# sdrobert/pydrobert-pytorch

Hardware: AMD Instinct MI355X
Metric: utterances/sec (N=4096,T=512) error_rate+ctc_beam at 1/2/4/8 GPU (higher is better)
Workload: dtype f32

## Files before the change

pydrobert-pytorch_amd/csrc/ctc_frame.hpp:

```cpp
#pragma once
#include "wave_select.hpp"

namespace pdt {

#ifdef PDT_STAMPS
__device__ unsigned long long g_stamps[16];
__device__ unsigned long long *g_stamp_lds_dummy;
#define PDT_STAMP(ph)                                                        \
  do {                                                                       \
    const unsigned long long now_ = __builtin_readcyclecounter();           \
    pdt_stamp_acc[ph] += (unsigned)(now_ - stamp_last_);                     \
    stamp_last_ = now_;                                                      \
  } while (0)
#define PDT_STAMP_BEGIN unsigned long long stamp_last_ = __builtin_readcyclecounter()
#else
#define PDT_STAMP(ph) do {} while (0)
#define PDT_STAMP_BEGIN do {} while (0)
#endif

#ifdef PDT_STATS
__device__ unsigned long long g_stats[24];
#define PDT_STAT(i) do { if (lane_id() == 0) atomicAdd(&g_stats[i], 1ull); } while (0)
#else
#define PDT_STAT(i) do {} while (0)
#endif

#ifdef PDT_UTT_STATS
__device__ unsigned g_utt_stats[8192 * 4];
#define PDT_UTT(k, v) do { pdt_utt_acc[k] += (unsigned)(v); } while (0)
#else
#define PDT_UTT(k, v) do {} while (0)
#endif

constexpr int kMaxWidth = 32;

struct CtcArgs {
  const float *logits;
  int64_t lg_st, lg_sn, lg_sv;
  const int64_t *lens;
  int T, N, V, W, S;
  int64_t *y;
  int64_t *y_lens;
  float *y_probs;
  int2 *trie;
  int2 *ckpt;
  unsigned char *grow;
  int ckpt_shift, ckpt_count;
  int lds_per_wave, waves_per_wg;
  int exact_div;
  int no_lean_extra;
  int no_steady;
};

struct Beam {
  float nb, b;
  int last, len, node;
  unsigned isp;
  int origin = 0;
};

__device__ __forceinline__ u64 readlane_u64(u64 v, int l) {
  const unsigned lo = (unsigned)__builtin_amdgcn_readlane((int)(unsigned)v, l);
  const unsigned hi = (unsigned)__builtin_amdgcn_readlane((int)(unsigned)(v >> 32), l);
  return ((u64)hi << 32) | lo;
}
__device__ __forceinline__ float readlane_f(float v, int l) {
  return __int_as_float(__builtin_amdgcn_readlane(__float_as_int(v), l));
}
__device__ __forceinline__ float shfl_f(float v, int l) { return __int_as_float(shfl_i(__float_as_int(v), l)); }
__device__ __forceinline__ unsigned fresh_zero() {
  unsigned z;
  asm volatile("v_mov_b32 %0, 0" : "=v"(z));
  return z;
}

struct DenseCtx {
  const float *ext;
  int64_t ext_sk, ext_sv;
  const int64_t *y_prev;
  int64_t yp_ss, yp_sk;
  int S;
  int lists_ready;
  const float *etab = nullptr;
  int etab_stride = 0;
  const int16_t *y_prev16 = nullptr;
  const int *slot = nullptr;
  const int *list_id = nullptr;
  unsigned closed = 0u;
  const int *lpos = nullptr;
  int lpos_stride = 0;
};

__host__ __device__ inline int nxt_stride(int W) { return W * W < 128 ? 128 : W * W; }
__host__ __device__ inline int consumer_scratch_bytes(int W) {
  return (2 * nxt_stride(W) * 4 + (W > 0 ? W : 1) * 4 * 3 + 7) & ~7;
}

struct FrameLds {
  u64 *surv;
  int *tl_tok;
  float *tl_p;
  unsigned char *pos;
  unsigned *chm;
  int *info;
  int *nxt_old, *nxt_new;
  int list_len;
  float *hdr;
  int2 *trie_u = nullptr;
  float pl_in = 0.0f, pblank_in = 0.0f;
  static __host__ __device__ size_t bytes(int V, int W, int Kp, bool dense) {
    const int RS = W > Kp ? W : Kp;
    size_t b = (size_t)PDT_SURV_CAP * 8 + (size_t)(dense ? Kp : 1) * PDT_WAVE * 8;
    b += dense ? 0 : (size_t)((V + 15) & ~15);
    b += (size_t)RS * 4 + (size_t)2 * W * 4 + (dense ? 0 : (size_t)2 * W * W * 4);
    return (b + 15) & ~(size_t)15;
  }
  __device__ void carve(unsigned char *base, int V, int W, int Kp, bool dense) {
    const int RS = W > Kp ? W : Kp, L = dense ? Kp : 1;
    surv = reinterpret_cast<u64 *>(base);
    tl_tok = reinterpret_cast<int *>(surv + PDT_SURV_CAP);
    tl_p = reinterpret_cast<float *>(tl_tok + L * PDT_WAVE);
    chm = reinterpret_cast<unsigned *>(tl_p + L * PDT_WAVE);
    info = reinterpret_cast<int *>(chm + RS);
    nxt_old = info + 2 * W;
    nxt_new = nxt_old + (dense ? 0 : W * W);
    pos = reinterpret_cast<unsigned char *>(nxt_new + (dense ? 0 : W * W));
  }
};

__device__ __forceinline__ int ctc_list_len(int V, int W, int Kp) {
  const int K = min(W, Kp * (V + 1));
  return min(V, K + Kp);
}

template <bool LONG = false>
__device__ __forceinline__ void build_shared_list(const float *p, float inv, int V, int M, u64 *surv,
                                                  int *tl_tok, float *tl_p, unsigned char *pos,
                                                  const unsigned *lmax_in = nullptr,
                                                  unsigned *probe = nullptr, int probe_rank = 1) {
  const int lane = lane_id();
  const u64 tk = wave_top_sorted<LONG, true>(p, V, M, surv, lmax_in, probe, probe_rank);
  if (lane < M) {
    const int tok = (int)idx_of(tk);
    tl_tok[lane] = tok;
    tl_p[lane] = p[tok] * inv;
    pos[tok] = (unsigned char)lane;
  }
}

#if defined(PDT_STAMPS)
#define PDT_STAMP_PARAM , unsigned *pdt_stamp_acc
#define PDT_STAMP_ARG , pdt_stamp_acc
#elif defined(PDT_UTT_STATS)
#define PDT_STAMP_PARAM , unsigned *pdt_utt_acc
#define PDT_STAMP_ARG , pdt_utt_acc
#else
#define PDT_STAMP_PARAM
#define PDT_STAMP_ARG
#endif

template <bool DENSE, bool ROWLESS = false, bool TRIE = !DENSE>
__device__ __forceinline__ bool ctc_frame(Beam &bm, const float *p, const float inv, const int V,
                                          const int W, const int Kp, const int t,
                                          const int64_t n, const CtcArgs &a, const DenseCtx &dc,
                                          const FrameLds &L, int &new_src, int &new_tok,
                                          int &new_kind PDT_STAMP_PARAM) {
  int lane = lane_id();
  asm volatile("" : "+v"(lane));
  const bool live = lane < Kp;
  const int K = min(W, Kp * (V + 1));
  const int M = min(V, K + Kp);
  const int me = live ? lane : 0;
  PDT_STAMP_BEGIN;

  if (DENSE && !dc.lists_ready) {
    for (int k = 0; k < Kp; ++k) {
      const u64 tk = wave_top_sorted_strided<true>(dc.ext + k * dc.ext_sk, dc.ext_sv, V, M, L.surv);
      if (lane < M) {
        L.tl_tok[k * PDT_WAVE + lane] = (int)idx_of(tk);
        L.tl_p[k * PDT_WAVE + lane] = fkey_inv(key_of(tk));
      }
      wave_sync();
    }
  }
  PDT_STAMP(1);
  auto list_of = [&](const int k) -> int { return DENSE ? (dc.list_id ? dc.list_id[k] : k) : 0; };
  const int my_list = list_of(me);
  const int *mt = L.tl_tok + my_list * PDT_WAVE;

  static_assert(!(DENSE && ROWLESS), "the row-less form reads the shared list");
  const float p_blank = ROWLESS ? L.pblank_in : p[V] * inv;
  const int lastc = min(max(bm.last, 0), V - 1);
  const float pl = ROWLESS ? L.pl_in : p[lastc] * inv;
  const float e_last = DENSE ? (dc.etab ? dc.etab[my_list * dc.etab_stride + me] : dc.ext[me * dc.ext_sk + lastc * dc.ext_sv]) : pl;
  const float tot = bm.nb + bm.b;
  const float B = tot * p_blank;
  float NB = bm.nb * pl;
  const bool valid_beam = live && tot > -PDT_INF;
  wave_sync();

  const int c_list = (DENSE || ROWLESS) ? M : min(L.list_len, M);
  const bool full_list = DENSE || ROWLESS || c_list >= M;
  int jl = -1;
  u64 avail = 0ull;
// ... 482 lines not shown
  PDT_STAMP(3);
  const int srcl = new_kind >= 0 ? new_src : lane;
  float NB_s = NB, B_s = B;
  int last_s = lastc, len_s = bm.len, node_s = bm.node;
  unsigned isp_s = bm.isp;
  if (!steady_f) {
    NB_s = shfl_f(NB, srcl), B_s = shfl_f(B, srcl);
    last_s = shfl_i(lastc, srcl), len_s = shfl_i(bm.len, srcl), node_s = shfl_i(bm.node, srcl);
    isp_s = (unsigned)shfl_i((int)bm.isp, srcl);
  }
  const bool is_ext = new_kind == 0 || new_kind == 1;
  const bool is_valid = new_kind >= 0;
  Beam nw;
  nw.nb = !is_valid ? -PDT_INF : (is_ext ? new_mass : NB_s);
  nw.b = !is_valid ? -PDT_INF : (is_ext ? 0.0f : B_s);
  nw.last = !is_valid ? 0 : (is_ext ? new_tok : last_s);
  nw.len = !is_valid ? 0 : len_s + (is_ext ? 1 : 0);
  nw.node = !is_valid ? -1 : (is_ext ? t * W + lane : node_s);
  if (TRIE) nw.origin = steady_f ? bm.origin : shfl_i(bm.origin, srcl);
  if (TRIE && is_valid && is_ext)
    *reinterpret_cast<int2 *>(reinterpret_cast<char *>(L.trie_u) + (unsigned)(t * W + lane) * 8u) = make_int2(node_s, new_tok);

  PDT_STAMP(4);
  const int RS = W > Kp ? W : Kp;
  if (!steady_f) {
    if (lane < RS) L.chm[lane] = fresh_zero();
    wave_sync();
    if (is_valid) atomicOr(&L.chm[new_src], 1u << lane);
  }
  if (is_valid) {
    L.info[2 * lane] = new_tok;
    L.info[2 * lane + 1] = len_s | (new_src << 20) | ((is_ext ? 1 : 0) << 28);
  }
  wave_sync();
  PDT_STAMP(10);
  unsigned isp_new = 0u;
  bool need_walk = false;
  bool pairs_done = false;
#ifndef PDT_NO_PAIR_PREFIX
#ifndef PDT_PAIR_DENSE
#define PDT_PAIR_DENSE 8
#endif
  if (__builtin_expect(TRIE && W <= 16 && !a.no_lean_extra && __ballot(is_valid && __popc(isp_s) > PDT_PAIR_DENSE) != 0ull, 0)) {
    const int pa = lane & 15, pq = lane >> 4;
    const u64 vmask = __ballot(is_valid);
    const int a_tok = shfl_i(new_tok, pa);
    const int a_w = shfl_i(len_s | (new_src << 20) | ((is_ext ? 1 : 0) << 28) | ((is_valid ? 1 : 0) << 29), pa);
    const unsigned a_isp = (unsigned)shfl_i((int)isp_s, pa);
    const int a_len_s = a_w & 0xFFFFF, a_src = (a_w >> 20) & 0xFF;
    const bool a_ext = (a_w >> 28) & 1, a_valid = (a_w >> 29) & 1;
    const int a_len = a_len_s + (a_ext ? 1 : 0);
    unsigned bits = 0u, walks = 0u;
#pragma unroll
    for (int r = 0; r < 4; ++r) {
      const int b = 4 * r + pq;
      const int tok_b = L.info[2 * b], w1 = L.info[2 * b + 1];
      const int lenB = w1 & 0xFFFFF, src_b = (w1 >> 20) & 0xFF;
      const bool ext_b = (w1 >> 28) & 1;
      const int len_b = lenB + (ext_b ? 1 : 0);
      bool pref = a_valid && ((vmask >> b) & 1ull) && b != pa && ((a_isp >> src_b) & 1u) && !(a_len > len_b);
      int tok_at = -1;
      if (pref) tok_at = lenB > a_len_s ? L.nxt_old[a_src * W + src_b] : (ext_b ? tok_b : -1);
      pref = pref && !(a_ext && tok_at != a_tok);
      bool walk = false;
      if (pref && a_len < len_b) {
        int nx;
        if (!a_ext) {
          nx = tok_at;
        } else if (lenB == a_len_s + 1) {
          nx = tok_b;
        } else {
          nx = -(2 + b);
          walk = true;
        }
        L.nxt_new[pa * W + b] = nx;
      }
      const u64 m = __ballot(pref), wm = __ballot(walk);
      const unsigned lo = (unsigned)m >> pa, hi = (unsigned)(m >> 32) >> pa;
      bits |= ((lo & 1u) | ((lo >> 15) & 2u) | ((hi & 1u) << 2) | ((hi >> 13) & 8u)) << (4 * r);
      walks |= (unsigned)(wm | (wm >> 16) | (wm >> 32) | (wm >> 48));
    }
    if (is_valid) {
      isp_new = bits | (1u << lane);
      need_walk = (walks >> lane) & 1u;
    }
    pairs_done = true;
    wave_sync();
  }
#endif
  if (is_valid && !pairs_done) {
    unsigned cand = 0u;
    if (steady_f) cand = isp_s;
    else
      for (unsigned m = isp_s; m; m &= m - 1u) cand |= L.chm[__builtin_ctz(m)];
    cand &= ~(1u << lane);
    isp_new = 1u << lane;
    while (cand) {
      const int b = __builtin_ctz(cand);
      cand &= cand - 1u;
      const int tok_b = L.info[2 * b], w1 = L.info[2 * b + 1];
      const int lenB = w1 & 0xFFFFF, src_b = (w1 >> 20) & 0xFF;
      const bool ext_b = (w1 >> 28) & 1;
      const int len_b = lenB + (ext_b ? 1 : 0);
      if (nw.len > len_b) continue;
      int tok_at;
      if (lenB > len_s)
        tok_at = !TRIE ? (dc.y_prev16 ? (int)dc.y_prev16[(int64_t)len_s * dc.yp_ss + (dc.slot ? dc.slot[src_b] : src_b) * dc.yp_sk]
                                      : (int)dc.y_prev[(int64_t)len_s * dc.yp_ss + (dc.slot ? dc.slot[src_b] : src_b) * dc.yp_sk])
                       : L.nxt_old[new_src * W + src_b];
      else
        tok_at = ext_b ? tok_b : -1;
      if (is_ext && tok_at != new_tok) continue;
      isp_new |= 1u << b;
      if (TRIE && nw.len < len_b) {
        int nx;
        if (!is_ext) {
          nx = tok_at;
        } else if (lenB == len_s + 1) {
          nx = tok_b;
        } else {
          nx = -(2 + b);
          need_walk = true;
        }
        L.nxt_new[lane * W + b] = nx;
      }
    }
  }
  if (TRIE && __ballot(need_walk)) {
    __builtin_amdgcn_fence(__ATOMIC_RELEASE, "agent");
    for (int b = 0; b < K; ++b) {
      const int node_b = __builtin_amdgcn_readlane(node_s, b);
      const int lenB = __builtin_amdgcn_readlane(len_s, b);
      if (need_walk && ((isp_new >> b) & 1u) && L.nxt_new[lane * W + b] == -(2 + b)) {
        int node = node_b, depth = lenB, tok = -1;
        while (node >= 0) {
          const int2 *rec = a.trie + ((int64_t)n * a.T * W + node);
          const int par_ = __hip_atomic_load(&rec->x, __ATOMIC_RELAXED, __HIP_MEMORY_SCOPE_AGENT);
          tok = __hip_atomic_load(&rec->y, __ATOMIC_RELAXED, __HIP_MEMORY_SCOPE_AGENT);
          if (depth == nw.len + 1) break;
          node = par_;
          --depth;
        }
        L.nxt_new[lane * W + b] = tok;
      }
    }
  }
  nw.isp = isp_new;
  bm = nw;
  wave_sync();
  PDT_STAMP(5);
  return list_sufficed;
}

template <int JW = 4>
__device__ __forceinline__ void walk_trie_segments(const int2 *tab, const int nseg, const int W, const int2 *trie_u,
                                                   int64_t *y_n, const int64_t row_stride) {
  const int lane = lane_id();
  for (int base = 0; base < nseg; base += JW * PDT_WAVE) {
    int node[JW], ps[JW], stop[JW], col[JW];
#pragma unroll
    for (int j = 0; j < JW; ++j) {
      const int sg = base + j * PDT_WAVE + lane;
      node[j] = -1, ps[j] = -1, stop[j] = 0, col[j] = 0;
      if (sg < nseg) {
        const int c = sg / W;
        col[j] = sg - c * W;
        const int2 top = tab[sg];
        stop[j] = c > 0 ? tab[sg - W].y : 0;
        node[j] = top.x;
        ps[j] = top.y - 1;
      }
    }
    bool any = true;
    while (any) {
      any = false;
      u64 rec[JW];
      bool act[JW];
#pragma unroll
      for (int j = 0; j < JW; ++j) {
        act[j] = ps[j] >= stop[j] && node[j] >= 0;
        rec[j] = 0ull;
        if (act[j]) rec[j] = *reinterpret_cast<const u64 *>(trie_u + node[j]);
      }
#pragma unroll
      for (int j = 0; j < JW; ++j) {
        if (act[j]) {
          y_n[(int64_t)ps[j] * row_stride + col[j]] = (int64_t)(int)(unsigned)(rec[j] >> 32);
          node[j] = (int)(unsigned)rec[j];
          --ps[j];
          any = true;
        }
      }
    }
  }
}

}
```

pydrobert-pytorch_amd/csrc/ctc_search.hip:

```cpp
#include "ctc_ring.hpp"
#include "switches.hpp"

#include <cstdlib>

namespace pdt {

template <int P, int NT = -1, bool INREG = (P == 1), bool GROW = false, int WC = -1, int VC = -1, bool PAIR = false>
__global__ void __launch_bounds__(256, INREG ? 8 : 4)
ctc_search_kernel(const CtcArgs a, const RingLayout rl_arg) {
  static_assert(!INREG || P == 1, "the register-resident row pass is a one-producer form");
  static_assert((WC > 0 && VC > 0) ? (P == 1 && INREG && !GROW) : true, "compile-time shapes: the register-resident form");
  const RingLayout rl = (WC > 0 && VC > 0) ? ring_layout(VC, WC, PDT_RING_STAGES, PDT_UTT_PER_WG, 1) : rl_arg;
  static_assert(!GROW || !INREG, "rows in the workspace are a form of the generic row pass");
  static_assert(NT < 0 || INREG, "compile-time chunk counts belong to the register-resident row pass");
  extern __shared__ __align__(16) unsigned char smem[];
  const int lane = lane_id();
  const int wave = __builtin_amdgcn_readfirstlane((int)(threadIdx.x >> 6));
  const int u = wave / (P + 1);
  const int role = wave - u * (P + 1);
  const bool producer = role < P;
  const int64_t n_raw = (int64_t)xcd_remap(blockIdx.x, gridDim.x) * rl.utt_per_wg + u;
  const bool idle = u >= rl.utt_per_wg || n_raw >= a.N;
  const int64_t n = idle ? 0 : n_raw;
  const int V = VC > 0 ? VC : a.V, W = WC > 0 ? WC : a.W;
// ... 299 lines not shown
#pragma unroll
          for (int i = 0; i < kPrefetch; ++i) {
            if (i > nt) break;
            if (i < nt) {
              pre[i] = nrow[(int64_t)(i * PDT_WAVE) * lg_sv];
            } else if (i == nt) {
              if (in_row) pre[i] = nrow[(int64_t)(i * PDT_WAVE) * lg_sv];
            }
          }
        }
      } else {
        float mx = -PDT_INF;
#pragma unroll
        for (int i = 0; i < kPrefetch; ++i) {
          const int v = lane + i * PDT_WAVE;
          if (v <= V) {
            p[v] = pre[i];
            mx = fmaxf(mx, pre[i]);
          }
        }
        {
          const float *row = a.logits + (int64_t)t * a.lg_st + n * lg_sn;
          int v = lane + kPrefetch * PDT_WAVE;
          if constexpr (!INREG) {
            for (; v + (kBatch - 1) * PDT_WAVE <= V; v += kBatch * PDT_WAVE) {
              float x[kBatch];
#pragma unroll
              for (int i = 0; i < kBatch; ++i) x[i] = row[(int64_t)(v + i * PDT_WAVE) * lg_sv];
#pragma unroll
              for (int i = 0; i < kBatch; ++i) {
                p[v + i * PDT_WAVE] = x[i];
                mx = fmaxf(mx, x[i]);
              }
            }
            for (; v <= V; v += 8 * PDT_WAVE) {
              float x[8];
#pragma unroll
              for (int i = 0; i < 8; ++i)
                x[i] = v + i * PDT_WAVE <= V ? row[(int64_t)(v + i * PDT_WAVE) * lg_sv] : -PDT_INF;
#pragma unroll
              for (int i = 0; i < 8; ++i) {
                if (v + i * PDT_WAVE <= V) p[v + i * PDT_WAVE] = x[i];
                mx = fmaxf(mx, x[i]);
              }
            }
          }
          for (; v <= V; v += PDT_WAVE) {
            const float x = row[(int64_t)v * lg_sv];
            p[v] = x;
            mx = fmaxf(mx, x);
          }
        }
        if (t + P < Tn) {
          const float *nrow = a.logits + (int64_t)(t + P) * a.lg_st + n * lg_sn + (int64_t)lane * lg_sv;
#pragma unroll
          for (int i = 0; i < kPrefetch; ++i) {
            const int v = lane + i * PDT_WAVE;
            if (v <= V) pre[i] = nrow[(int64_t)(i * PDT_WAVE) * lg_sv];
          }
        }
        mx = wave_max_f(mx);
        {
          int v = lane;
          if constexpr (!INREG) {
            for (; v + 7 * PDT_WAVE <= V; v += 8 * PDT_WAVE) {
              float x[8];
#pragma unroll
              for (int i = 0; i < 8; ++i) x[i] = p[v + i * PDT_WAVE];
#pragma unroll
              for (int i = 0; i < 8; ++i) {
                const float e = exp_nonpos(x[i] - mx);
                p[v + i * PDT_WAVE] = e;
                s += e;
              }
            }
          }
          for (; v <= V; v += PDT_WAVE) {
            const float e = exp_nonpos(p[v] - mx);
            p[v] = e;
            s += e;
          }
        }
      }
      s = wave_sum_f(s);
      wave_sync();
      const int M = ctc_list_len(V, W, (t == 0 && !(WC > 0 && VC > 0 && VC + 1 >= WC)) ? 1 : W);
      const float inv0 = __builtin_amdgcn_rcpf(s);
      float inv = __builtin_fmaf(__builtin_fmaf(-s, inv0, 1.0f), inv0, inv0);
      if (VC <= 0 && a.exact_div) {
        for (int v = lane; v <= V; v += PDT_WAVE) p[v] = p[v] / s;
        wave_sync();
        inv = 1.0f;
      }
      int Ml = M;
      if (short_ok && nshort >= kShortMin && nshort <= kShortMax) {
        PDT_STAT(1);
        const unsigned sk = lane < nshort ? surv32[lane] : 0u;
        unsigned st = nshort <= 16 ? row_sort_desc<unsigned>(sk) : half_wave_sort_desc<unsigned>(sk);
        const unsigned st_next = (unsigned)__builtin_amdgcn_mov_dpp((int)st, 0x130, 0xf, 0xf, true);
        int tok = 511 - (int)(st & 511u);
        if (__ballot(lane + 1 < nshort && (st >> 9) == (st_next >> 9)) != 0ull) {
          const int tk0 = 511 - (int)((lane < nshort ? surv32[lane] : 0u) & 511u);
          const u64 tk = half_wave_sort_desc<u64>(lane < nshort ? pack_key(fkey_nonneg(p[tk0]), (unsigned)tk0) : 0ull);
          tok = (int)idx_of(tk);
        }
        Ml = min(nshort, M);
        if (lane < Ml) {
          tl_tok[lane] = tok;
          slot_p(sl)[lane] = p[tok] * inv;
          pos[tok] = (unsigned char)lane;
        }
        const float step = fmaxf(fabsf(thr_off) * 0.03125f, 1e-3f);
        thr_off += nshort > kShortHi ? step : (nshort < kShortLo ? -step : 0.0f);
      } else {
        PDT_STAT(nshort > kShortMax ? 3 : 2);
        unsigned probe = 0u;
        build_shared_list<!INREG>(p, inv, V, M, surv, tl_tok, slot_p(sl), pos, INREG ? &lmax : nullptr,
                                  &probe, kProbeRank);
        if (short_ok) thr_off = mx_of_row + __logf(fkey_nonneg_inv(probe)) - mean;
      }
      PDT_STAT(0);
      if (lane == 0) {
        hdr[0] = inv;
        hdr[2] = __int_as_float(Ml);
      }
      wave_sync();
      if (lane == 0)
        __hip_atomic_store(&ready[P == 1 ? 0 : sl], t + 1, __ATOMIC_RELEASE, __HIP_MEMORY_SCOPE_WORKGROUP);
    }
    return;
  }

#ifndef PDT_NO_PRIO
  __builtin_amdgcn_s_setprio(PDT_CONSUMER_PRIO);
#endif
  FrameLds L;
  L.surv = surv;
  L.trie_u = a.trie + (int64_t)n * a.T * W;
  L.nxt_old = reinterpret_cast<int *>(cs);
  L.nxt_new = L.nxt_old + nxt_stride(W);
  L.chm = reinterpret_cast<unsigned *>(L.nxt_new + nxt_stride(W));
  L.info = reinterpret_cast<int *>(L.chm + W);
  Beam bm;
  bm.nb = lane == 0 ? 0.0f : -PDT_INF;
  bm.b = lane == 0 ? 1.0f : -PDT_INF;
  bm.last = 0;
  bm.len = 0;
  bm.node = -1;
  bm.isp = lane == 0 ? 1u : 0u;
  bm.origin = lane;
  constexpr bool kFullFromStart = WC > 0 && VC > 0 && VC + 1 >= WC;
  int Kp = kFullFromStart ? WC : 1;
  int fail_score = 0, full_mode = 0;
  const int ckpt_shift = (WC > 0 && VC > 0) ? 5 : a.ckpt_shift;
#ifdef PDT_STAMPS
  unsigned pdt_stamp_acc[14] = {0};
#endif
  int sl = 0;
#ifdef PDT_UTT_STATS
  const unsigned long long utt_t0_ = __builtin_readcyclecounter();
  unsigned pdt_utt_acc[4] = {0, 0, 0, 0};
#endif
  for (int t = 0; t < Tn; ++t, sl = sl + 1 == NS ? 0 : sl + 1) {
    PDT_STAMP_BEGIN;
#ifdef PDT_UTT_STATS
    const unsigned long long w0_ = __builtin_readcyclecounter();
#endif
    if (__hip_atomic_load(&ready[P == 1 ? 0 : sl], __ATOMIC_ACQUIRE, __HIP_MEMORY_SCOPE_WORKGROUP) <= t) {
#ifndef PDT_NO_PRIO
      __builtin_amdgcn_s_setprio(0);
#endif
      do {
        __builtin_amdgcn_s_sleep(PDT_SPIN_SLEEP);
      } while (__hip_atomic_load(&ready[P == 1 ? 0 : sl], __ATOMIC_ACQUIRE, __HIP_MEMORY_SCOPE_WORKGROUP) <= t);
#ifndef PDT_NO_PRIO
      __builtin_amdgcn_s_setprio(PDT_CONSUMER_PRIO);
#endif
    }
    PDT_STAMP(0);
#if defined(PDT_UTT_STATS) && !defined(PDT_UTT_REASONS)
    PDT_UTT(3, (__builtin_readcyclecounter() - w0_) >> 4);
#endif
    L.tl_tok = slot_tok(sl);
    L.tl_p = slot_p(sl);
    L.pos = slot_pos(sl);
    L.hdr = slot_hdr(sl);
    L.list_len = __float_as_int(slot_hdr(sl)[2]);
    const float s = slot_hdr(sl)[0];
    int ns, nt, nk;
    int lane_t = lane;
#ifndef PDT_SKIP_CONSUMER
    bool enough = true;
    if (!(readlane_f(bm.nb + bm.b, 0) == 0.0f)) {
      enough = ctc_frame<false>(bm, slot_row(sl), s, V, W, Kp, t, n, a, DenseCtx{}, L, ns, nt, nk PDT_STAMP_ARG);
      int *tmp = L.nxt_old;
      L.nxt_old = L.nxt_new;
      L.nxt_new = tmp;
      if (!kFullFromStart) Kp = W;
    }
    const int enough_s = __builtin_amdgcn_readfirstlane(enough ? 1 : 0);
    fail_score = enough_s ? max(fail_score - 1, 0) : min(fail_score + 1, 32);
    const int wf = fail_score > 16 ? 1 : (fail_score < 4 ? 0 : full_mode);
    if (wf != full_mode) {
      full_mode = wf;
      asm volatile("" : "+v"(lane_t));
      if (lane_t == 0) __hip_atomic_store(want_full, wf, __ATOMIC_RELAXED, __HIP_MEMORY_SCOPE_WORKGROUP);
    }
#else
    ns = nt = nk = 0; (void)s;
    if (!kFullFromStart) Kp = W;
#endif
    asm volatile("" : "+v"(lane_t));
    if (lane_t == 0) __hip_atomic_store(consumed, t + 1, __ATOMIC_RELEASE, __HIP_MEMORY_SCOPE_WORKGROUP);
    if (((t + 1) & ((1 << ckpt_shift) - 1)) == 0) {
      const int c = ((t + 1) >> ckpt_shift) - 1;
      if (lane_t < W)
        a.ckpt[((int64_t)n * a.ckpt_count + c) * W + lane_t] = make_int2(bm.node, bm.len | (bm.origin << 24));
      bm.origin = lane_t;
    }
  }

#ifdef PDT_UTT_STATS
  if (lane == 0 && n < 8192) {
    g_utt_stats[n * 4 + 0] = (unsigned)((__builtin_readcyclecounter() - utt_t0_) >> 4);
    for (int k = 1; k < 4; ++k) g_utt_stats[n * 4 + k] = pdt_utt_acc[k];
  }
#endif
#ifdef PDT_STAMPS
  if (lane == 0)
    for (int i = 0; i < 14; ++i) atomicAdd(&g_stamps[i], (unsigned long long)pdt_stamp_acc[i]);
  unsigned long long stamp_last_ = __builtin_readcyclecounter();
#endif
  if (lane < W) {
    a.y_probs[n * W + lane] = bm.nb + bm.b;
    a.y_lens[n * W + lane] = bm.len;
  }
  __builtin_amdgcn_fence(__ATOMIC_RELEASE, "workgroup");
  __builtin_amdgcn_fence(__ATOMIC_ACQUIRE, "agent");
#ifndef PDT_SKIP_WALK
  {
    const int C = Tn >> ckpt_shift;
    int2 *tab = reinterpret_cast<int2 *>(ring);
    if (lane < W) {
      const bool ok = bm.node >= 0;
      tab[C * W + lane] = make_int2(bm.node, bm.len);
      int cur = bm.origin;
      for (int c = C - 1; c >= 0; --c) {
        const int2 rec = a.ckpt[((int64_t)n * a.ckpt_count + c) * W + cur];
        const int nd = rec.x, lo = rec.y;
        tab[c * W + lane] = ok ? make_int2(nd, lo & 0xFFFFFF) : make_int2(-1, 0);
        cur = lo >> 24;
      }
    }
    wave_sync();
#ifdef PDT_STAMPS
    unsigned long long st1_ = __builtin_readcyclecounter();
    if (lane == 0) atomicAdd(&g_stamps[11], st1_ - stamp_last_);
#endif
    walk_trie_segments(tab, (C + 1) * W, W, a.trie + (int64_t)n * a.T * W, a.y + n * W, (int64_t)a.N * W);
#ifdef PDT_STAMPS
    unsigned long long st2_ = __builtin_readcyclecounter();
    if (lane == 0) atomicAdd(&g_stamps[12], st2_ - st1_);
#endif
    int lmin = lane < W ? bm.len : 0x7fffffff;
    for (int off = 32; off > 0; off >>= 1) lmin = min(lmin, shfl_i(lmin, lane ^ off));
    for (int f = lmin * W + lane; f < a.S * W; f += PDT_WAVE) {
      const int pos = f / W, k = f - pos * W;
      if (pos >= tab[C * W + k].y) a.y[((int64_t)pos * a.N + n) * W + k] = 0;
    }
  }
#endif
#ifdef PDT_STAMPS
  if (lane == 0) atomicAdd(&g_stamps[6], __builtin_readcyclecounter() - stamp_last_);
#endif
}

template <int P, int NT = -1, bool INREG = (P == 1), bool GROW = false, int WC = -1, int VC = -1, bool PAIR = false>
static int launch_ctc_search_p(const CtcArgs &a, const RingLayout &rl, hipStream_t stream) {
  const size_t smem = (size_t)rl.utt_bytes * rl.utt_per_wg;
  if (const int rc = set_lds(ctc_search_kernel<P, NT, INREG, GROW, WC, VC, PAIR>, smem)) return rc;
  const unsigned grid = (unsigned)((a.N + rl.utt_per_wg - 1) / rl.utt_per_wg);
  hipLaunchKernelGGL((ctc_search_kernel<P, NT, INREG, GROW, WC, VC, PAIR>), dim3(grid), dim3(64 * (P + 1) * rl.utt_per_wg), smem,
                     stream, a, rl);
  return (int)hipGetLastError();
}

__host__ inline int ckpt_shift_for(int T, int W, const RingLayout &rl) {
  const size_t ring = (size_t)rl.slot_bytes * rl.nstage;
  int sh = 5;
  while (((size_t)(T >> sh) + 1) * W * sizeof(int2) > ring) ++sh;
  return sh;
}

struct CtcPlan {
  int producers, nstage, utt_per_wg, inreg;
};
__host__ inline int plan_ctc_search(int V, int W, CtcPlan *plan, RingLayout *rl) {
  if (W < 1 || W > kMaxWidth) return PDT_E_TOO_LONG;
  const size_t soft_cap = 64 * 1024, hard_cap = 160 * 1024;
  if (V + 1 > 8 * PDT_WAVE) {
    *rl = ring_layout(V, W, 4, 1, 3);
    if ((size_t)rl->utt_bytes * 4 <= hard_cap) return *plan = CtcPlan{3, 4, 1, 0}, PDT_OK;

    *rl = ring_layout(V, W, 3, 1, 3);
    if ((size_t)rl->utt_bytes <= hard_cap) return *plan = CtcPlan{3, 3, 1, 0}, PDT_OK;
    *rl = ring_layout(V, W, 4, 1, 3, true);
    return *plan = CtcPlan{3, 4, 1, 2}, PDT_OK;
  }
  int nstage = PDT_RING_STAGES, upw = PDT_UTT_PER_WG;
  *rl = ring_layout(V, W, nstage, upw, 1);
  while ((size_t)rl->utt_bytes * upw > soft_cap && (upw > 1 || nstage > 2)) {
    if (upw > 1) upw = 1; else nstage = 2;
    *rl = ring_layout(V, W, nstage, upw, 1);
  }
  if ((size_t)rl->utt_bytes * upw > hard_cap) return PDT_E_TOO_LONG;
  return *plan = CtcPlan{1, nstage, upw, 1}, PDT_OK;
}

bool ctc_rowreg_applies(int V, int W);
void ctc_rowreg_plan(int V, int W, int32_t *plan5);
int launch_ctc_rowreg(CtcArgs a, hipStream_t stream);

int launch_ctc_search(const CtcArgs &a, const CtcPlan &plan, const RingLayout &rl, hipStream_t stream) {
  if (plan.inreg == 2) return launch_ctc_search_p<3, -1, false, true>(a, rl, stream);
  if (plan.producers == 3) return launch_ctc_search_p<3>(a, rl, stream);
#ifndef PDT_NO_V256
  {
    const RingLayout c = ring_layout(256, 16, PDT_RING_STAGES, PDT_UTT_PER_WG, 1);
    if (a.V == 256 && a.W == 16 && a.ckpt_shift == 5 && !a.exact_div && !a.no_lean_extra && a.lg_sv == 1 && a.lg_sn == 257 && c.nstage == rl.nstage && c.utt_per_wg == rl.utt_per_wg && c.utt_bytes == rl.utt_bytes &&
        c.slot_bytes == rl.slot_bytes) {
      if (switches().ctc_pair != 0 && rl.nstage == 4) return launch_ctc_search_p<1, 4, true, false, 16, 256, true>(a, rl, stream);
      return launch_ctc_search_p<1, 4, true, false, 16, 256>(a, rl, stream);
    }
  }
#endif
#ifndef PDT_NO_WIDTH16
  if (a.V / PDT_WAVE == 4 && a.W == 16) return launch_ctc_search_p<1, 4, true, false, 16>(a, rl, stream);
#endif
  if (a.V / PDT_WAVE == 4) return launch_ctc_search_p<1, 4>(a, rl, stream);
  return launch_ctc_search_p<1>(a, rl, stream);
}

}

extern "C" {

static int64_t ctc_trie_bytes(int64_t T, int64_t N, int64_t width) {
  return ((T + T / 32 + 1) * N * width * (int64_t)sizeof(int2) + 255) & ~(int64_t)255;
}

int64_t pdt_ctc_prefix_search_workspace_bytes(int64_t T, int64_t N, int64_t V, int64_t width) {
  if (T < 0 || N < 0 || V < 1 || width < 1 || V >= (1 << 30)) return 0;
  int64_t bytes = ctc_trie_bytes(T, N, width) + 16;
  pdt::CtcPlan plan;
  pdt::RingLayout rl;
  if (pdt::plan_ctc_search((int)V, (int)(width > pdt::kMaxWidth ? pdt::kMaxWidth : width), &plan, &rl) == PDT_OK &&
      rl.row_global)
    bytes += N * (int64_t)rl.nstage * rl.g_slot_bytes;
  return bytes;
}

int pdt_ctc_prefix_search_plan(int64_t V, int64_t width, int32_t *plan5) {
  int32_t *plan4 = plan5;
  if (V < 1 || width < 1 || !plan5) return PDT_E_ARG;
  if (V >= (1 << 30)) return PDT_E_TOO_LONG;
  pdt::CtcPlan plan;
  pdt::RingLayout rl;
  const int rc = pdt::plan_ctc_search((int)V, (int)width, &plan, &rl);
  if (rc != PDT_OK) return rc;
  plan4[0] = plan.producers; plan4[1] = plan.nstage; plan4[2] = plan.utt_per_wg; plan4[3] = plan.inreg;
  plan5[4] = 0;
  if (pdt::ctc_rowreg_applies((int)V, (int)width)) pdt::ctc_rowreg_plan((int)V, (int)width, plan5);
  return PDT_OK;
}

int pdt_ctc_prefix_search(const float *logits, int64_t T, int64_t N, int64_t V, int64_t lg_st,
                          int64_t lg_sn, int64_t lg_sv, const int64_t *lens, int64_t width,
                          int64_t S, int64_t *y, int64_t *y_lens, float *y_probs,
                          void *workspace, void *stream) {
  using namespace pdt;
  if (T < 0 || N < 0 || V < 1 || width < 1 || S < 0) return PDT_E_ARG;
  if (N == 0) return PDT_OK;
  if (!y_lens || !y_probs || (T > 0 && (!logits || !workspace)) || (S > 0 && !y)) return PDT_E_ARG;
  if (width > kMaxWidth) return PDT_E_TOO_LONG;
  if (T * width >= (1ll << 31) || V >= (1 << 30) || N >= (1ll << 31) || T >= (1 << 24)) return PDT_E_TOO_LONG;
  CtcArgs a{};
  a.logits = logits; a.lg_st = lg_st; a.lg_sn = lg_sn; a.lg_sv = lg_sv;
  a.lens = lens;
  a.T = (int)T; a.N = (int)N; a.V = (int)V; a.W = (int)width; a.S = (int)S;
  a.y = y; a.y_lens = y_lens; a.y_probs = y_probs;
  a.trie = reinterpret_cast<int2 *>(workspace);
  a.ckpt = a.trie + T * N * width;
  a.grow = reinterpret_cast<unsigned char *>(workspace) + ctc_trie_bytes(T, N, width);
  a.exact_div = switches().ctc_exact_div == 1 ? 1 : 0;
  a.no_lean_extra = switches().ctc_lean_extra == 0 ? 1 : 0;
  a.no_steady = switches().ctc_steady == 0 ? 1 : 0;
  if (ctc_rowreg_applies(a.V, a.W) && lg_sv == 1) return launch_ctc_rowreg(a, (hipStream_t)stream);
  CtcPlan plan;
  RingLayout rl;
  const int rc = plan_ctc_search(a.V, a.W, &plan, &rl);
  if (rc != PDT_OK) return rc;
  a.ckpt_shift = ckpt_shift_for((int)T, (int)width, rl);
  a.ckpt_count = (int)(T >> a.ckpt_shift) + 1;
  return launch_ctc_search(a, plan, rl, (hipStream_t)stream);
}

}

#ifdef PDT_STATS
extern "C" int pdt_debug_read_stats(unsigned long long *host24, int reset) {
  hipError_t e = hipMemcpyFromSymbol(host24, HIP_SYMBOL(pdt::g_stats), sizeof(unsigned long long) * 24);
  if (e == hipSuccess && reset) {
    unsigned long long z[24] = {0};
    e = hipMemcpyToSymbol(HIP_SYMBOL(pdt::g_stats), z, sizeof(z));
  }
  return (int)e;
}
#endif

#ifdef PDT_UTT_STATS
extern "C" int pdt_debug_read_utt_stats(unsigned *host, int count, int reset) {
  hipError_t e = hipMemcpyFromSymbol(host, HIP_SYMBOL(pdt::g_utt_stats), sizeof(unsigned) * 4 * (size_t)count);
  if (e == hipSuccess && reset) {
    static unsigned z[8192 * 4];
    e = hipMemcpyToSymbol(HIP_SYMBOL(pdt::g_utt_stats), z, sizeof(z));
  }
  return (int)e;
}
#endif

#ifdef PDT_STAMPS
extern "C" int pdt_debug_read_stamps(unsigned long long *host16, int reset) {
  hipError_t e = hipMemcpyFromSymbol(host16, HIP_SYMBOL(pdt::g_stamps), sizeof(unsigned long long) * 16);
  if (e == hipSuccess && reset) {
    unsigned long long z[16] = {0};
    e = hipMemcpyToSymbol(HIP_SYMBOL(pdt::g_stamps), z, sizeof(z));
  }
  return (int)e;
}
#endif
```

pydrobert-pytorch_amd/csrc/pdt_api.hip:

```cpp
#include <cmath>
#include <algorithm>
#include <cstdlib>

#include "lev_launch.hpp"
#include "switches.hpp"
#include <cstring>
#include <mutex>

namespace pdt {
static bool costs_exact_in_f32(float ins, float del, float sub, int64_t R, int64_t H) {
  const float c[3] = {ins, del, sub};
  float mx = 0.0f;
  for (float v : c) {
    if (!std::isfinite(v)) return false;
    mx = std::fmax(mx, std::fabs(v));
  }
  for (int q = 0; q <= 20; ++q) {
    bool ok = true;
    for (float v : c) {
      const float s = std::ldexp(v, q);
      ok = ok && (s == std::floor(s));
    }
    if (ok) {
      const double bound = (double)(R + H + 2) * (double)std::ldexp(mx, q);
      return bound < 16777216.0;
    }
  }
  return false;
}

static bool bitpar_enabled() { return switches().lev_bitpar != 0; }

static bool oc_bitpar_enabled() { return switches().oc_bitpar != 0; }

namespace {
struct SwitchName {
  const char *name;
  int Switches::*field;
  int deft;
};
const SwitchName kSwitchNames[] = {
    {"PDT_LEV_BITPAR", &Switches::lev_bitpar, 1},         {"PDT_OC_BITPAR", &Switches::oc_bitpar, 1},
    {"PDT_CTC_EXACT_DIV", &Switches::ctc_exact_div, 0},   {"PDT_CTC_ROWREG", &Switches::ctc_rowreg, 1},
    {"PDT_STEP_WIDE", &Switches::step_wide, 0},           {"PDT_CTC_LEAN_EXTRA", &Switches::ctc_lean_extra, 1},
    {"PDT_CTC_PAIR", &Switches::ctc_pair, 1},             {"PDT_STEP_FLAT", &Switches::step_flat, 1},
    {"PDT_CTC_STEADY", &Switches::ctc_steady, 1},
};
}

Switches &switches() {
  static Switches s = [] {
    Switches v{};
    for (const SwitchName &n : kSwitchNames) {
      const char *e = std::getenv(n.name);
      v.*(n.field) = (e && e[0]) ? std::atoi(e) : n.deft;
    }
    return v;
  }();
  return s;
}

namespace {
std::mutex g_kept_mu;
const void *g_kept[16] = {};
unsigned g_kept_next = 0;
}
static void kept_tables_forget(const void *ws) {
  std::lock_guard<std::mutex> lock(g_kept_mu);
  for (const void *&e : g_kept)
    if (e == ws) e = nullptr;
}
static void kept_tables_note(const void *ws) {
  kept_tables_forget(ws);
  std::lock_guard<std::mutex> lock(g_kept_mu);
  g_kept[g_kept_next++ % 16] = ws;
}
static bool kept_tables_has(const void *ws) {
  std::lock_guard<std::mutex> lock(g_kept_mu);
  for (const void *e : g_kept)
    if (e == ws) return true;
  return false;
}

static int fill_common(LevArgs &a, const int64_t *ref, int64_t R, int64_t ref_st, int64_t ref_sn,
                       const int64_t *hyp, int64_t H, int64_t hyp_st, int64_t hyp_sn, int64_t N,
                       int has_eos, int64_t eos, int include_eos, float ins, float del, float sub) {
  if (R < 0 || H < 0 || N < 0) return PDT_E_ARG;
  if (N > 0 && ((R > 0 && !ref) || (H > 0 && !hyp))) return PDT_E_ARG;
  if (R > (1 << 28) || H > (1 << 28) || N > (1ll << 31) - 1) return PDT_E_TOO_LONG;
  a = LevArgs{};
  a.ref = ref; a.hyp = hyp;
  a.ref_st = ref_st; a.ref_sn = ref_sn; a.hyp_st = hyp_st; a.hyp_sn = hyp_sn;
  a.R = (int)R; a.H = (int)H; a.N = (int)N;
  a.has_eos = has_eos; a.eos = eos; a.include_eos = include_eos;
  a.ins = ins; a.del = del; a.sub = sub; a.mult = 1.0f;
  return PDT_OK;
}
}

extern "C" {

int pdt_amd_abi_version(void) { return 14; }

int pdt_amd_set_switch(const char *name, int value) {
  if (!name) return PDT_E_ARG;
  for (const pdt::SwitchName &n : pdt::kSwitchNames)
    if (std::strcmp(n.name, name) == 0) return pdt::switches().*(n.field) = value, PDT_OK;
  return PDT_E_ARG;
}

int pdt_amd_get_switch(const char *name, int *value) {
  if (!name || !value) return PDT_E_ARG;
  for (const pdt::SwitchName &n : pdt::kSwitchNames)
    if (std::strcmp(n.name, name) == 0) return *value = pdt::switches().*(n.field), PDT_OK;
  return PDT_E_ARG;
}

int64_t pdt_lev_workspace_bytes(int64_t R, int64_t H, int64_t N) {
  if (R < 0 || H < 0 || N <= 0) return 0;
  int64_t need = 0;
  if (pdt::bitpar_enabled()) {
    const pdt::BitparPlan p = pdt::plan_bitpar(H, R, N);
    if (p.ok) need = (int64_t)p.total;
  }
  if (R > 64 * 32) need = std::max(need, pdt::lev_workgroup_ws_per_utt(R, H, nullptr) * N);
  return need;
}

static int lev_entry(const int64_t *ref, int64_t R, int64_t ref_st, int64_t ref_sn, const int64_t *hyp,
                     int64_t H, int64_t hyp_st, int64_t hyp_sn, int64_t N, int has_eos, int64_t eos,
                     int include_eos, float ins_cost, float del_cost, float sub_cost, int norm, int mode,
                     int exclude_last, float padding, int return_mistakes, float *out, int64_t out_sh,
                     int64_t out_sn, int64_t *ref_lens_out, int64_t *hyp_lens_out, int32_t *status,
                     void *workspace, int64_t workspace_bytes, void *stream, pdt::LevTables tables) {
  using namespace pdt;
  if (mode != PDT_MODE_FINAL && mode != PDT_MODE_PREFIX) return PDT_E_ARG;
  if (exclude_last && mode != PDT_MODE_PREFIX) return PDT_E_ARG;
  if (exclude_last && H == 0) return PDT_E_ARG;
  if (N > 0 && !out) return PDT_E_ARG;
  float mult = 1.0f;
  if (ins_cost == del_cost && del_cost == sub_cost && sub_cost > 0.0f) {
    if (!return_mistakes) mult = ins_cost;
    ins_cost = del_cost = sub_cost = 1.0f;
    return_mistakes = 0;
  }
  LevArgs a;
  int rc = fill_common(a, ref, R, ref_st, ref_sn, hyp, H, hyp_st, hyp_sn, N, has_eos, eos,
                       include_eos, ins_cost, del_cost, sub_cost);
  if (rc != PDT_OK) return rc;
  if (N == 0) return PDT_OK;
  a.mult = mult;
  a.norm = norm; a.mode = mode; a.exclude_last = exclude_last; a.count = return_mistakes;
  a.padding = padding;
  a.out = out; a.out_sh = out_sh; a.out_sn = out_sn;
  a.ref_lens_out = ref_lens_out; a.hyp_lens_out = hyp_lens_out; a.status = status;
  if (!return_mistakes && !costs_exact_in_f32(ins_cost, del_cost, sub_cost, R, H)) {
    if (R > 64 * 32) return launch_lev_workgroup(a, true, workspace, workspace_bytes, (hipStream_t)stream);
    return launch_lev_rowsync(a, true, (hipStream_t)stream);
  }
  if (!return_mistakes && ins_cost == 1.0f && del_cost == 1.0f && sub_cost == 1.0f && workspace &&
      bitpar_enabled()) {
    const BitparPlan p = plan_bitpar(H, R, N);
    if (p.ok && (int64_t)p.total <= workspace_bytes) {
      if (tables == kTablesGiven && !kept_tables_has(workspace)) tables = kTablesOwn;
      rc = launch_lev_bitpar(a, p, workspace, (hipStream_t)stream, tables);
      if (tables == kTablesKeep || (tables == kTablesOwn && !p.fused)) kept_tables_note(workspace);
      else if (tables == kTablesOwn) kept_tables_forget(workspace);
      return rc;
    }
  }
  return launch_lev_skewed(a, (hipStream_t)stream);
}

int pdt_lev(const int64_t *ref, int64_t R, int64_t ref_st, int64_t ref_sn, const int64_t *hyp,
            int64_t H, int64_t hyp_st, int64_t hyp_sn, int64_t N, int has_eos, int64_t eos,
            int include_eos, float ins_cost, float del_cost, float sub_cost, int norm, int mode,
            int exclude_last, float padding, int return_mistakes, float *out, int64_t out_sh,
            int64_t out_sn, int64_t *ref_lens_out, int64_t *hyp_lens_out, int32_t *status,
            void *workspace, int64_t workspace_bytes, void *stream) {
  return lev_entry(ref, R, ref_st, ref_sn, hyp, H, hyp_st, hyp_sn, N, has_eos, eos, include_eos, ins_cost,
                   del_cost, sub_cost, norm, mode, exclude_last, padding, return_mistakes, out, out_sh, out_sn,
                   ref_lens_out, hyp_lens_out, status, workspace, workspace_bytes, stream, pdt::kTablesOwn);
}

int pdt_lev_keep(const int64_t *ref, int64_t R, int64_t ref_st, int64_t ref_sn, const int64_t *hyp,
                 int64_t H, int64_t hyp_st, int64_t hyp_sn, int64_t N, int has_eos, int64_t eos,
                 int include_eos, float ins_cost, float del_cost, float sub_cost, int norm, int mode,
                 int exclude_last, float padding, int return_mistakes, float *out, int64_t out_sh,
                 int64_t out_sn, int64_t *ref_lens_out, int64_t *hyp_lens_out, int32_t *status,
                 void *workspace, int64_t workspace_bytes, void *stream) {
  return lev_entry(ref, R, ref_st, ref_sn, hyp, H, hyp_st, hyp_sn, N, has_eos, eos, include_eos, ins_cost,
                   del_cost, sub_cost, norm, mode, exclude_last, padding, return_mistakes, out, out_sh, out_sn,
                   ref_lens_out, hyp_lens_out, status, workspace, workspace_bytes, stream, pdt::kTablesKeep);
}

int pdt_lev_classified(const int64_t *ref, int64_t R, int64_t ref_st, int64_t ref_sn, const int64_t *hyp,
                       int64_t H, int64_t hyp_st, int64_t hyp_sn, int64_t N, int has_eos, int64_t eos,
                       int include_eos, float ins_cost, float del_cost, float sub_cost, int norm, int mode,
                       int exclude_last, float padding, int return_mistakes, float *out, int64_t out_sh,
// ... 62 lines not shown
```

pydrobert-pytorch_amd/csrc/switches.hpp:

```cpp
#pragma once

namespace pdt {

struct Switches {
  int lev_bitpar;
  int oc_bitpar;
  int ctc_exact_div;
  int ctc_rowreg;
  int step_wide;
  int ctc_pair;
  int step_flat;
  int ctc_lean_extra;
  int ctc_steady;
};

Switches &switches();

}
```

pydrobert-pytorch_amd/pydrobert_amd/switches.py:

```python

import contextlib
import ctypes
import os

from . import _cabi

_HOST_DEFAULTS = {
    "PDT_LEV_CACHE": 0,
    "PDT_CTC_LM_FUSED": 1,
    "PDT_CTC_LM_TABLE": 1,
    "PDT_BEAM_FUSED": 1,
    "PDT_BEAM_SEARCH": 1,
    "PDT_BEAM_TABLE": 1,
    "PDT_CHECK_INVARIANTS": 0,
    "PDT_WALK_TABLE": 1,
}
_NATIVE = (
    "PDT_LEV_BITPAR", "PDT_OC_BITPAR", "PDT_CTC_EXACT_DIV", "PDT_CTC_ROWREG", "PDT_STEP_WIDE",
    "PDT_CTC_LEAN_EXTRA", "PDT_CTC_PAIR", "PDT_STEP_FLAT", "PDT_CTC_STEADY",
)


def _from_env(name, default):
    raw = os.environ.get(name, "")
    try:
        return int(raw) if raw != "" else default
    except ValueError:
        return default


_values = {name: _from_env(name, deft) for name, deft in _HOST_DEFAULTS.items()}


def names():
    return tuple(_HOST_DEFAULTS) + _NATIVE


def get(name: str) -> int:
    if name in _values:
        return _values[name]
    if name in _NATIVE:
        out = ctypes.c_int(0)
        _cabi.check(_cabi.lib().pdt_amd_get_switch(name.encode(), ctypes.addressof(out)), "pdt_amd_get_switch")
        return out.value
    raise KeyError(name)


def set(name: str, value: int) -> None:
    if name in _values:
        _values[name] = int(value)
    elif name in _NATIVE:
        _cabi.check(_cabi.lib().pdt_amd_set_switch(name.encode(), int(value)), "pdt_amd_set_switch")
    else:
        raise KeyError(name)


@contextlib.contextmanager
def override(**kw):
    old = {k: get(k) for k in kw}
    try:
        for k, v in kw.items():
            set(k, v)
        yield
    finally:
        for k, v in old.items():
            set(k, v)
```

Baseline: 2.291 million.

## Process two steady CTC beam frames per wave step with half-wave rows

Adds a fast path for the paired-producer CTC beam search that handles two consecutive frames in one pass. It uses the two 16-lane halves of the wave for the two rows, exchanging values through permlane16 swaps, and checks with DPP max reductions and ballots that the top-K selection is trivially ordered. When that check fails it falls back to the single-frame path, and a backoff gate skips later attempts after repeated failures. The aim is to halve per-frame sync and selection overhead in steady stretches, at the cost of extra speculative work whenever the check fails and a hardcoded W=16 shape.

```diff
diff --git a/pydrobert-pytorch_amd/csrc/ctc_frame.hpp b/pydrobert-pytorch_amd/csrc/ctc_frame.hpp
--- a/pydrobert-pytorch_amd/csrc/ctc_frame.hpp
+++ b/pydrobert-pytorch_amd/csrc/ctc_frame.hpp
@@ -50,6 +50,7 @@
   int exact_div;
   int no_lean_extra;
   int no_steady;
+  int no_twoframe;
 };
 
 struct Beam {
@@ -838,6 +839,101 @@
   return list_sufficed;
 }
 
+template <int V, int W>
+__device__ __forceinline__ bool ctc_two_steady_frames(Beam &bm, unsigned char *slot_t, const int slot_bytes,
+                                                      const int row_floats, const int pos_bytes, const int t,
+                                                      int2 *trie_u) {
+  static_assert(W == 16 && V >= 2 * W && V + 1 >= W, "two rows of 16 beam entries, lists of K + K' = 32 entries");
+  constexpr int K = W, M = 2 * W;
+  int lane = lane_id();
+  asm volatile("" : "+v"(lane));
+  if (__ballot((lane < W) & (!(bm.nb + bm.b > -PDT_INF) | ((bm.isp & ~(1u << lane)) != 0u))) != 0ull) {
+    PDT_STAT(19);
+    return false;
+  }
+  const bool row1 = lane >= W;
+  const unsigned char *sb = slot_t + (row1 ? slot_bytes : 0);
+  const float *p = reinterpret_cast<const float *>(sb);
+  const int *tl_tok = reinterpret_cast<const int *>(sb + row_floats * 4);
+  const float *tl_p = reinterpret_cast<const float *>(tl_tok + PDT_WAVE);
+  const unsigned char *pos = reinterpret_cast<const unsigned char *>(tl_p + PDT_WAVE);
+  const float *hdr = reinterpret_cast<const float *>(pos + pos_bytes);
+  const float inv = hdr[0];
+  const int c_list = min(__float_as_int(hdr[2]), M);
+  const bool full_list = c_list >= M;
+  const unsigned have = c_list >= 32 ? ~0u : ((1u << c_list) - 1u);
+  float nb = bm.nb, b = bm.b;
+  int last = bm.last;
+  {
+    const int lastc = min(max(last, 0), V - 1);
+    const unsigned q = pos[lastc];
+    const unsigned av0 = have & ~(unsigned)(1ull << (q & 63u));
+    const int j0 = av0 ? __builtin_ctz(av0) : 0;
+    const int tok0 = tl_tok[j0];
+    const float x = (nb + b) * tl_p[j0];
+    const auto rx = __builtin_amdgcn_permlane16_swap(__float_as_uint(x), __float_as_uint(x), false, false);
+    const auto rt = __builtin_amdgcn_permlane16_swap((unsigned)tok0, (unsigned)tok0, false, false);
+    nb = row1 ? __uint_as_float(rx[0]) : nb;
+    b = row1 ? 0.0f : b;
+    last = row1 ? (int)rt[0] : last;
+  }
+  const int lastc = min(max(last, 0), V - 1);
+  const float p_blank = p[V] * inv;
+  const float pl = p[lastc] * inv;
+  const unsigned q = pos[lastc];
+  const float tot = nb + b;
+  const float B = tot * p_blank;
+  const float NB = nb * pl;
+  const float m1 = b * pl;
+  const float m2 = NB + B;
+  const unsigned av0 = have & ~(unsigned)(1ull << (q & 63u)), av1 = av0 & (av0 - 1u);
+  const bool bound1 = !full_list && av1 == 0u;
+  const int j0 = av0 ? __builtin_ctz(av0) : 0;
+  const int j1 = av1 ? __builtin_ctz(av1) : (bound1 ? c_list - 1 : 0);
+  const int tok0 = tl_tok[j0];
+  const float p0 = tl_p[j0], p1 = tl_p[j1];
+  const float x0 = tot * p0;
+  const bool real0 = av0 != 0u;
+  const unsigned key0 = real0 ? fkey_nonneg(x0) : 0u;
+  const unsigned key1 = (av1 != 0u || bound1) ? fkey_nonneg(tot * p1) + (bound1 ? 1u : 0u) : 0u;
+  const unsigned key2 = fkey_nonneg(m1), key3 = fkey_nonneg(m2);
+  const unsigned key_next = (unsigned)__builtin_amdgcn_mov_dpp((int)key0, 0x101, 0xf, 0xf, true);
+  const unsigned real_m = (unsigned)__ballot(real0);
+  const unsigned desc = (unsigned)__ballot(key0 >= key_next) | 0x80008000u;
+  unsigned v = max(max(key1, key2), key3);
+  v = max(v, (unsigned)dpp_or<PDT_DPP_ROW_SHR(1)>((int)v, 0));
+  v = max(v, (unsigned)dpp_or<PDT_DPP_ROW_SHR(2)>((int)v, 0));
+  v = max(v, (unsigned)dpp_or<PDT_DPP_ROW_SHR(4), 0xf, 0xe>((int)v, 0));
+  v = max(v, (unsigned)dpp_or<PDT_DPP_ROW_SHR(8), 0xf, 0xc>((int)v, 0));
+  const unsigned rest_a = (unsigned)__builtin_amdgcn_readlane((int)v, K - 1);
+  const unsigned rest_b = (unsigned)__builtin_amdgcn_readlane((int)v, W + K - 1);
+  const unsigned kth_a = (unsigned)__builtin_amdgcn_readlane((int)key0, K - 1);
+  const unsigned kth_b = (unsigned)__builtin_amdgcn_readlane((int)key0, W + K - 1);
+  if (!((real_m & desc) == ~0u && kth_a > max(rest_a, 64u) && kth_b > max(rest_b, 64u))) {
+    PDT_STAT(19);
+    return false;
+  }
+  PDT_STAT(18);
+#ifdef PDT_STATS
+  {
+    const unsigned bm_ = (unsigned)__ballot(bound1);
+    if ((bm_ & 0xFFFFu) != 0u) PDT_STAT(17);
+    if ((bm_ >> 16) != 0u) PDT_STAT(17);
+  }
+#endif
+  if (lane < 2 * W)
+    *reinterpret_cast<int2 *>(reinterpret_cast<char *>(trie_u) + (unsigned)(t * W + lane) * 8u) =
+        make_int2(row1 ? t * W + lane - W : bm.node, tok0);
+  const auto bx = __builtin_amdgcn_permlane16_swap(__float_as_uint(x0), __float_as_uint(x0), false, false);
+  const auto bt = __builtin_amdgcn_permlane16_swap((unsigned)tok0, (unsigned)tok0, false, false);
+  bm.nb = __uint_as_float(bx[1]);
+  bm.b = 0.0f;
+  bm.last = (int)bt[1];
+  bm.len += 2;
+  bm.node = (t + 1) * W + lane;
+  return true;
+}
+
 template <int JW = 4>
 __device__ __forceinline__ void walk_trie_segments(const int2 *tab, const int nseg, const int W, const int2 *trie_u,
                                                    int64_t *y_n, const int64_t row_stride) {
diff --git a/pydrobert-pytorch_amd/csrc/ctc_search.hip b/pydrobert-pytorch_amd/csrc/ctc_search.hip
--- a/pydrobert-pytorch_amd/csrc/ctc_search.hip
+++ b/pydrobert-pytorch_amd/csrc/ctc_search.hip
@@ -475,6 +475,7 @@
   constexpr bool kFullFromStart = WC > 0 && VC > 0 && VC + 1 >= WC;
   int Kp = kFullFromStart ? WC : 1;
   int fail_score = 0, full_mode = 0;
+  int two_gate = 0;
   const int ckpt_shift = (WC > 0 && VC > 0) ? 5 : a.ckpt_shift;
 #ifdef PDT_STAMPS
   unsigned pdt_stamp_acc[14] = {0};
@@ -513,6 +514,34 @@
     int ns, nt, nk;
     int lane_t = lane;
 #ifndef PDT_SKIP_CONSUMER
+    auto list_feedback = [&](const int enough_s) {
+      fail_score = enough_s ? max(fail_score - 1, 0) : min(fail_score + 1, 32);
+      const int wf = fail_score > 16 ? 1 : (fail_score < 4 ? 0 : full_mode);
+      if (wf != full_mode) {
+        full_mode = wf;
+        asm volatile("" : "+v"(lane_t));
+        if (lane_t == 0) __hip_atomic_store(want_full, wf, __ATOMIC_RELAXED, __HIP_MEMORY_SCOPE_WORKGROUP);
+      }
+    };
+    bool single = true;
+    if constexpr (PAIR) {
+      if ((t & 1) == 0 && t + 1 < Tn && !a.no_steady && !a.no_twoframe && !(readlane_f(bm.nb + bm.b, 0) == 0.0f)) {
+        if ((two_gate & 0xFF) != 0) {
+          --two_gate;
+        } else if (ctc_two_steady_frames<VC, WC>(bm, ring + sl * rl.slot_bytes, rl.slot_bytes, rl.row_floats, rl.pos_bytes, t, L.trie_u)) {
+          list_feedback(1);
+          list_feedback(1);
+          ++t;
+          ++sl;
+          single = false;
+          two_gate = 0;
+        } else {
+          const int lvl = min((two_gate >> 8) + 1, 5);
+          two_gate = (lvl << 8) | (lvl < 3 ? 0 : (1 << lvl) - 4);
+        }
+      }
+    }
+    if (single) {
     bool enough = true;
     if (!(readlane_f(bm.nb + bm.b, 0) == 0.0f)) {
       enough = ctc_frame<false>(bm, slot_row(sl), s, V, W, Kp, t, n, a, DenseCtx{}, L, ns, nt, nk PDT_STAMP_ARG);
@@ -521,13 +550,7 @@
       L.nxt_new = tmp;
       if (!kFullFromStart) Kp = W;
     }
-    const int enough_s = __builtin_amdgcn_readfirstlane(enough ? 1 : 0);
-    fail_score = enough_s ? max(fail_score - 1, 0) : min(fail_score + 1, 32);
-    const int wf = fail_score > 16 ? 1 : (fail_score < 4 ? 0 : full_mode);
-    if (wf != full_mode) {
-      full_mode = wf;
-      asm volatile("" : "+v"(lane_t));
-      if (lane_t == 0) __hip_atomic_store(want_full, wf, __ATOMIC_RELAXED, __HIP_MEMORY_SCOPE_WORKGROUP);
+    list_feedback(__builtin_amdgcn_readfirstlane(enough ? 1 : 0));
     }
 #else
     ns = nt = nk = 0; (void)s;
@@ -718,6 +741,7 @@
   a.exact_div = switches().ctc_exact_div == 1 ? 1 : 0;
   a.no_lean_extra = switches().ctc_lean_extra == 0 ? 1 : 0;
   a.no_steady = switches().ctc_steady == 0 ? 1 : 0;
+  a.no_twoframe = (switches().ctc_twoframe == 0 || a.no_steady) ? 1 : 0;
   if (ctc_rowreg_applies(a.V, a.W) && lg_sv == 1) return launch_ctc_rowreg(a, (hipStream_t)stream);
   CtcPlan plan;
   RingLayout rl;
diff --git a/pydrobert-pytorch_amd/csrc/pdt_api.hip b/pydrobert-pytorch_amd/csrc/pdt_api.hip
--- a/pydrobert-pytorch_amd/csrc/pdt_api.hip
+++ b/pydrobert-pytorch_amd/csrc/pdt_api.hip
@@ -44,7 +44,7 @@
     {"PDT_CTC_EXACT_DIV", &Switches::ctc_exact_div, 0},   {"PDT_CTC_ROWREG", &Switches::ctc_rowreg, 1},
     {"PDT_STEP_WIDE", &Switches::step_wide, 0},           {"PDT_CTC_LEAN_EXTRA", &Switches::ctc_lean_extra, 1},
     {"PDT_CTC_PAIR", &Switches::ctc_pair, 1},             {"PDT_STEP_FLAT", &Switches::step_flat, 1},
-    {"PDT_CTC_STEADY", &Switches::ctc_steady, 1},
+    {"PDT_CTC_STEADY", &Switches::ctc_steady, 1},         {"PDT_CTC_TWOFRAME", &Switches::ctc_twoframe, 1},
 };
 }
 
diff --git a/pydrobert-pytorch_amd/csrc/switches.hpp b/pydrobert-pytorch_amd/csrc/switches.hpp
--- a/pydrobert-pytorch_amd/csrc/switches.hpp
+++ b/pydrobert-pytorch_amd/csrc/switches.hpp
@@ -12,6 +12,7 @@
   int step_flat;
   int ctc_lean_extra;
   int ctc_steady;
+  int ctc_twoframe;
 };
 
 Switches &switches();
diff --git a/pydrobert-pytorch_amd/pydrobert_amd/switches.py b/pydrobert-pytorch_amd/pydrobert_amd/switches.py
--- a/pydrobert-pytorch_amd/pydrobert_amd/switches.py
+++ b/pydrobert-pytorch_amd/pydrobert_amd/switches.py
@@ -18,6 +18,7 @@
 _NATIVE = (
     "PDT_LEV_BITPAR", "PDT_OC_BITPAR", "PDT_CTC_EXACT_DIV", "PDT_CTC_ROWREG", "PDT_STEP_WIDE",
     "PDT_CTC_LEAN_EXTRA", "PDT_CTC_PAIR", "PDT_STEP_FLAT", "PDT_CTC_STEADY",
+    "PDT_CTC_TWOFRAME",
 )
 
 
```

After: 2.417 million (median of 6 runs). 1.06x the previous value.
